# logan-pearce/olpefit

Hardware: NVIDIA B200
Metric: pixel_model_evals_per_sec (higher is better)
Workload: dtype f32

## Files before the change

### olpefit_b200/csrc/lapf.cu

```cuda
#include <algorithm>
#include <charconv>
#include <cmath>
#include <cstdarg>
#include <cstdio>
#include <cstdlib>
#include <cstring>
#include <limits>
#include <new>
#include <string>
#include <vector>

#include <cuda.h>

#include "../../include/lapf.h"
#include "lapf_device.cuh"

using namespace lapf;

static thread_local char g_err[512] = "";

static int fail(int code, const char* fmt, ...) {
    va_list ap;
    va_start(ap, fmt);
    vsnprintf(g_err, sizeof(g_err), fmt, ap);
// ... 410 lines not shown
        if (u == next_rec) {
            if (lane <= P && tw == 0) {
                const size_t mi = (size_t)wl * (P + 1) + lane;
                const double v = (lane == P) ? chi_c : p;
                const double dl = v - a.shift[mi];
                if (a.chain) {
                    const size_t ci = ((size_t)row * a.n_walkers + wl) * (P + 1) + lane;
                    if (a.chain_f32) static_cast<float*>(a.chain)[ci] = (float)dl; else static_cast<double*>(a.chain)[ci] = v;
                }
                atomicAdd(&a.moments[2 * mi], dl);
                atomicAdd(&a.moments[2 * mi + 1], dl * dl);
            }
            if (a.sk_hist) {
                double xy[2 * NB];
#pragma unroll
                for (int j = 0; j < 2 * NB; ++j) xy[j] = shfl_f64(p, j);
                if (lane == 0 && tw == 0) record_sketch<NB>(a, wl, frame, xy);
            }
            ++row;
            next_rec += a.thin;
        }
    }

    if (tw == 0) {
        if (lane < P) st[lane] = p;
        if (lane == P) st[P] = chi_c;
        if (lane == 0) a.exps[wl] += n_exps;
    }
}

template <int NB, int NX, int NY, int NW, int MINB, int TEAM>
__global__ void __launch_bounds__(NW * 32, MINB) gibbs_kernel(const __grid_constant__ RunArgs a) {
    static_assert(NW % TEAM == 0 && (TEAM == 1 || NW / TEAM <= 15), "teams must tile the CTA (named barriers 1..15)");
    extern __shared__ __align__(128) unsigned char smem_raw[];
    __shared__ WarpScratch scratch[NW];
    __shared__ double team_part[NW / TEAM][2 * TEAM];
    __shared__ uint64_t bar;
    float* sd = reinterpret_cast<float*>(smem_raw);
    float* sw = sd + NX * NY;
    float* rt = sw + NX * NY;
    const int warp = threadIdx.x >> 5, lane = threadIdx.x & 31;

    if (threadIdx.x == 0) mbar_init(&bar, 1);
    __syncthreads();

    const int i0 = (int)(((int64_t)a.n_items * blockIdx.x) / gridDim.x);
    const int i1 = (int)(((int64_t)a.n_items * (blockIdx.x + 1)) / gridDim.x);
    int cur_frame = -1;
    uint32_t phase = 0;
    for (int it = i0; it < i1; ++it) {
        const int f = a.item_frame[it];
        if (f != cur_frame) {
            __syncthreads();
            if (threadIdx.x == 0) {
                constexpr uint32_t kBytes = NX * NY * sizeof(float);
                fence_proxy_async();
                mbar_expect_tx(&bar, 2 * kBytes);
                tma_bulk_g2s(sd, a.data + (size_t)f * NX * NY, kBytes, &bar);
                tma_bulk_g2s(sw, a.weight + (size_t)f * NX * NY, kBytes, &bar);
            }
            mbar_wait(&bar, phase);
            phase ^= 1u;
            cur_frame = f;
            prep_stamp(sd, sw, NX * NY);
            __syncthreads();
        }
        const int team = warp / TEAM, tw = warp % TEAM;
        if (team < a.item_count[it]) {
            using S = Scratch<NB, NX, NY, TEAM>;
            float* base = rt + team * (TEAM > 1 ? S::TEAM_FLOATS : S::FLOATS);
            run_walker<NB, NX, NY, TEAM>(a, sd, sw, scratch[warp], base + (TEAM > 1 ? tw * S::TAB : 0), base + TEAM * S::TAB,
                                         team_part[team], team, tw, a.walker_of[a.item_first[it] + team], f, lane);
        }
    }
}

template <int NB, int NX, int NY, int LW, int TM, int WPP>
__device__ __forceinline__ void run_batch(const RunArgs& a, const float* sd, const float* sw, float* rt, float* img,
                                          int wl, int nl, int la, int frame0, int frame1, int slot, int lane,
                                          uint32_t tmem, uint32_t slot_cols) {
    using L = Layout<NB>;
    using I = CoefImg<NB, Geo<NX>::PANELS>;
    constexpr int P = L::P;
    const bool mine = wl >= 0;
    const uint64_t gid = (uint64_t)(a.id_base + (int64_t)wl * a.id_stride);
    const bool two = TM == 1 && frame1 >= 0;
    const int ox0 = a.origin[2 * frame0], oy0 = a.origin[2 * frame0 + 1];
    const int ox1 = two ? a.origin[2 * frame1] : ox0, oy1 = two ? a.origin[2 * frame1 + 1] : oy0;
    double* st = a.state + (size_t)(mine ? wl : 0) * (P + 1);
    double chi_c = mine ? st[P] : 0.0;

    const int n_upd = (int)a.n_updates;
    int next_rec = (int)min(a.next_record - a.t0 - 1, (int64_t)0x7fffffff);
    int row = 0;
    unsigned long long n_exps = 0;

#pragma unroll 1
    for (int u = 0; u < n_upd; ++u) {
        int k = 0;
        double nv = 0.0, lnu = 0.0;
        bool skip = false;
        if (mine) {
            const Draw dr = make_draw(a.seed, gid, (uint64_t)(a.t0 + u), P);
            const double oxd = (double)((two && slot) ? ox1 : ox0), oyd = (double)((two && slot) ? oy1 : oy0);
            k = dr.k;
            lnu = dr.lnu;
            const double wz = __dmul_rn(a.widths[k], dr.z);
            const bool is_log = (a.log_mask >> k) & 1u;
            double v[P];
#pragma unroll
            for (int j = 0; j < P; ++j) v[j] = st[j];
            double pk = v[0];
#pragma unroll
            for (int j = 1; j < P; ++j) pk = (j == k) ? v[j] : pk;
            nv = is_log ? (pk < 0.0 ? nan("") : __dmul_rn(pk, exp10(wz))) : __dadd_rn(pk, wz);
#pragma unroll
            for (int j = 0; j < P; ++j) v[j] = (j == k) ? nv : v[j];
            double fl = v[2 * NB];
#pragma unroll
            for (int j = 2 * NB + 1; j < P; ++j) fl = (j == a.floor_index) ? v[j] : fl;
            Coef<NB> cf;
            coef_from_vector<NB>(cf, v, fl, oxd, oyd);
            set_fast_serial<NB, NX, NY>(cf);
            if (a.plain) cf.fast = false;
            if (NX >= 64 && a.cull) set_cull_serial<NB, NX, NY>(cf); else no_cull<NB, NX, NY>(cf);
            skip = nv != nv;
            if (skip && WPP > 1) cf.fast = true;
            store_coef<NB, Geo<NX>::PANELS>(img + lane * I::STRIDE, cf, slot | (skip ? 2 : 0));
        }
        __syncwarp();

        double chi_t = 0.0;
        if constexpr (WPP == 1) {
#pragma unroll 1
            for (int i = 0; i < nl; ++i) {
                Coef<NB> cf;
                int sl = 0;
                load_coef<NB, Geo<NX>::PANELS>(cf, img + i * I::STRIDE, &sl);
                if (sl & 2) continue;
                unsigned e_upd = 0;
                const double c = warp_chi2<NB, NX, NY, false, true, 1, TM>(cf, rt, sd, sw, nullptr, lane, 0, &e_upd,
                                                                           TM == 1 ? tmem + (uint32_t)(sl & 1) * slot_cols : tmem);
                if (lane == i) { chi_t = c; n_exps += e_upd; }
            }
        } else {
#pragma unroll 1
            for (int seg = 0; seg < 2; ++seg) {
                const int i0 = seg ? la : 0, i1 = seg ? nl : la;
#pragma unroll 1
                for (int i = i0; i < i1; i += 2) {
                    const int mine_i = min(i + (lane >> 4), i1 - 1);
                    Coef<NB> cf;
                    int sl = 0;
                    load_coef<NB, 1>(cf, img + mine_i * I::STRIDE, &sl);
                    if (__all_sync(kFull, (sl & 2) != 0)) continue;
                    sl = __shfl_sync(kFull, sl, 0) & 1;
                    unsigned e_upd = 0;
                    const double c = warp_chi2_pair<NB, NX, NY, false, true, TM>(cf, rt, sd, sw, nullptr, lane, &e_upd,
                                                                                 tmem + (uint32_t)sl * slot_cols);
                    const double c0 = shfl_f64(c, 0), c1 = shfl_f64(c, 16);
                    const unsigned e0 = __shfl_sync(kFull, e_upd, 0), e1 = __shfl_sync(kFull, e_upd, 16);
                    if (lane == i) { chi_t = c0; n_exps += e0; }
                    if (lane == i + 1 && i + 1 < i1) { chi_t = c1; n_exps += e1; }
                }
            }
        }
        __syncwarp();

        if (mine) {
            if (skip) chi_t = nan("");
            if (a.outside) {
                double fl = st[a.floor_index];
                if (k == a.floor_index) fl = nv;
                chi_t += outside_chi2(a.outside, (two && slot) ? frame1 : frame0, fl);
            }
            const bool acc = lnu < -0.5 * (chi_t - chi_c);
            atomicAdd(&a.tries[(size_t)wl * P + k], 1u);
            if (acc) {
                atomicAdd(&a.accepts[(size_t)wl * P + k], 1u);
                st[k] = nv;
                chi_c = chi_t;
            }
        }
        if (u == next_rec) {
            if (mine) {
#pragma unroll 1
                for (int j = 0; j <= P; ++j) {
                    const size_t mi = (size_t)wl * (P + 1) + j;
                    const double v = (j == P) ? chi_c : st[j];
                    const double dl = v - a.shift[mi];
                    if (a.chain) {
                        const size_t ci = ((size_t)row * a.n_walkers + wl) * (P + 1) + j;
                        if (a.chain_f32) static_cast<float*>(a.chain)[ci] = (float)dl; else static_cast<double*>(a.chain)[ci] = v;
                    }
                    atomicAdd(&a.moments[2 * mi], dl);
                    atomicAdd(&a.moments[2 * mi + 1], dl * dl);
                }
                if (a.sk_hist) {
                    double xy[2 * NB];
#pragma unroll
                    for (int j = 0; j < 2 * NB; ++j) xy[j] = st[j];
                    record_sketch<NB>(a, wl, (two && slot) ? frame1 : frame0, xy);
                }
                if (a.probe) {
                    double* pb = a.probe + ((size_t)row * a.n_walkers + wl) * 3;
                    pb[0] = (double)k; pb[1] = nv; pb[2] = chi_t;
                }
            }
            ++row;
            next_rec += a.thin;
        }
    }
    if (mine) {
        st[P] = chi_c;
        a.exps[wl] += n_exps;
    }
// ... 1349 lines not shown
```

### olpefit_b200/csrc/lapf_device.cuh

```cuda
#pragma once
#ifndef LAPF_LOOP_UNROLL
#define LAPF_LOOP_UNROLL 2
#endif
#include <cstdint>
#include <cuda_runtime.h>

namespace lapf {

constexpr float kLog2e = 1.4426950408889634f;
constexpr int kLoopUnroll = LAPF_LOOP_UNROLL;
constexpr unsigned kFull = 0xffffffffu;

template <int NB>
struct Layout {
    static constexpr int NOBJ = NB;
    static constexpr int P = 3 * NB + 10;
    static constexpr int K = 2 * NB;
    static constexpr int I_DX = 2 * NB, I_DY = 2 * NB + 1;
    static constexpr int I_AMP = 2 * NB + 2;
    static constexpr int I_RATIO = 3 * NB + 2, I_BKGD = 3 * NB + 3;
    static constexpr int I_SX = 3 * NB + 4, I_SY = 3 * NB + 5, I_SX2 = 3 * NB + 6, I_SY2 = 3 * NB + 7;
    static constexpr int I_TH = 3 * NB + 8, I_TH2 = 3 * NB + 9;
};

__device__ __forceinline__ float ex2_approx(float x) {
    float y;
    asm("ex2.approx.ftz.f32 %0, %1;" : "=f"(y) : "f"(x));
    return y;
}

__device__ __forceinline__ double shfl_f64(double v, int src) {
    int lo = __double2loint(v), hi = __double2hiint(v);
    lo = __shfl_sync(kFull, lo, src);
    hi = __shfl_sync(kFull, hi, src);
    return __hiloint2double(hi, lo);
}

__device__ __forceinline__ double shfl_xor_f64(double v, int mask) {
    int lo = __double2loint(v), hi = __double2hiint(v);
    lo = __shfl_xor_sync(kFull, lo, mask);
    hi = __shfl_xor_sync(kFull, hi, mask);
    return __hiloint2double(hi, lo);
}

__device__ __forceinline__ double warp_sum_f64(double v) {
#pragma unroll
    for (int off = 16; off >= 1; off >>= 1) v += shfl_xor_f64(v, off);
    return v;
}

__device__ __forceinline__ uint32_t smem_u32(const void* p) {
    return static_cast<uint32_t>(__cvta_generic_to_shared(p));
}
__device__ __forceinline__ void mbar_init(uint64_t* bar, uint32_t count) {
    asm volatile("mbarrier.init.shared::cta.b64 [%0], %1;" ::"r"(smem_u32(bar)), "r"(count));
    asm volatile("fence.mbarrier_init.release.cluster;" ::: "memory");
}
__device__ __forceinline__ void mbar_expect_tx(uint64_t* bar, uint32_t bytes) {
    asm volatile("mbarrier.arrive.expect_tx.shared::cta.b64 _, [%0], %1;" ::"r"(smem_u32(bar)), "r"(bytes)
                 : "memory");
}
__device__ __forceinline__ void mbar_wait(uint64_t* bar, uint32_t parity) {
    asm volatile(
        "{\n\t"
        ".reg .pred p;\n\t"
        "WAIT_%=:\n\t"
        "mbarrier.try_wait.parity.shared::cta.b64 p, [%0], %1;\n\t"
        "@p bra DONE_%=;\n\t"
        "bra WAIT_%=;\n\t"
        "DONE_%=:\n\t"
        "}" ::"r"(smem_u32(bar)),
        "r"(parity)
        : "memory");
}
__device__ __forceinline__ void tma_bulk_g2s(void* dst_smem, const void* src_gmem, uint32_t bytes,
                                             uint64_t* bar) {
    asm volatile(
        "cp.async.bulk.shared::cluster.global.mbarrier::complete_tx::bytes [%0], [%1], %2, [%3];" ::"r"(
            smem_u32(dst_smem)),
        "l"(src_gmem), "r"(bytes), "r"(smem_u32(bar))
        : "memory");
}
__device__ __forceinline__ void fence_proxy_async() {
    asm volatile("fence.proxy.async.shared::cta;" ::: "memory");
}

__device__ __forceinline__ void tmem_alloc(uint32_t* slot_in_smem, uint32_t ncols) {
    asm volatile("tcgen05.alloc.cta_group::1.sync.aligned.shared::cta.b32 [%0], %1;" ::"r"(smem_u32(slot_in_smem)), "r"(ncols)
                 : "memory");
    asm volatile("tcgen05.relinquish_alloc_permit.cta_group::1.sync.aligned;" ::: "memory");
}
__device__ __forceinline__ void tmem_dealloc(uint32_t base, uint32_t ncols) {
    asm volatile("tcgen05.dealloc.cta_group::1.sync.aligned.b32 %0, %1;" ::"r"(base), "r"(ncols) : "memory");
}
__device__ __forceinline__ void tmem_fence_before_sync() { asm volatile("tcgen05.fence::before_thread_sync;" ::: "memory"); }
__device__ __forceinline__ void tmem_fence_after_sync() { asm volatile("tcgen05.fence::after_thread_sync;" ::: "memory"); }
__device__ __forceinline__ void tmem_wait_st() { asm volatile("tcgen05.wait::st.sync.aligned;" ::: "memory"); }

__device__ __forceinline__ void tmem_st16(uint32_t addr, const float (&v)[16]) {
    asm volatile("tcgen05.st.sync.aligned.32x32b.x16.b32 [%0], {%1,%2,%3,%4,%5,%6,%7,%8,%9,%10,%11,%12,%13,%14,%15,%16};"
                 ::"r"(addr), "r"(__float_as_uint(v[0])), "r"(__float_as_uint(v[1])), "r"(__float_as_uint(v[2])),
                   "r"(__float_as_uint(v[3])), "r"(__float_as_uint(v[4])), "r"(__float_as_uint(v[5])),
                   "r"(__float_as_uint(v[6])), "r"(__float_as_uint(v[7])), "r"(__float_as_uint(v[8])),
                   "r"(__float_as_uint(v[9])), "r"(__float_as_uint(v[10])), "r"(__float_as_uint(v[11])),
                   "r"(__float_as_uint(v[12])), "r"(__float_as_uint(v[13])), "r"(__float_as_uint(v[14])),
                   "r"(__float_as_uint(v[15]))
                 : "memory");
}
__device__ __forceinline__ void tmem_ld16_issue(uint32_t addr, uint32_t (&r)[16]) {
    asm volatile("tcgen05.ld.sync.aligned.32x32b.x16.b32 {%0,%1,%2,%3,%4,%5,%6,%7,%8,%9,%10,%11,%12,%13,%14,%15}, [%16];"
                 : "=r"(r[0]), "=r"(r[1]), "=r"(r[2]), "=r"(r[3]), "=r"(r[4]), "=r"(r[5]), "=r"(r[6]), "=r"(r[7]),
                   "=r"(r[8]), "=r"(r[9]), "=r"(r[10]), "=r"(r[11]), "=r"(r[12]), "=r"(r[13]), "=r"(r[14]), "=r"(r[15])
                 : "r"(addr));
}
__device__ __forceinline__ void tmem_st8(uint32_t addr, const float (&v)[8]) {
    asm volatile("tcgen05.st.sync.aligned.32x32b.x8.b32 [%0], {%1,%2,%3,%4,%5,%6,%7,%8};"
                 ::"r"(addr), "r"(__float_as_uint(v[0])), "r"(__float_as_uint(v[1])), "r"(__float_as_uint(v[2])),
                   "r"(__float_as_uint(v[3])), "r"(__float_as_uint(v[4])), "r"(__float_as_uint(v[5])),
                   "r"(__float_as_uint(v[6])), "r"(__float_as_uint(v[7]))
                 : "memory");
}
__device__ __forceinline__ void tmem_ld8_issue(uint32_t addr, uint32_t (&r)[16]) {
    asm volatile("tcgen05.ld.sync.aligned.32x32b.x8.b32 {%0,%1,%2,%3,%4,%5,%6,%7}, [%8];"
                 : "=r"(r[8]), "=r"(r[9]), "=r"(r[10]), "=r"(r[11]), "=r"(r[12]), "=r"(r[13]), "=r"(r[14]), "=r"(r[15])
                 : "r"(addr));
}
__device__ __forceinline__ void tmem_ld8_wait(uint32_t (&r)[16]) {
    asm volatile("tcgen05.wait::ld.sync.aligned;"
                 : "+r"(r[8]), "+r"(r[9]), "+r"(r[10]), "+r"(r[11]), "+r"(r[12]), "+r"(r[13]), "+r"(r[14]), "+r"(r[15]));
}
__device__ __forceinline__ void tmem_ld16_wait(uint32_t (&r)[16]) {
    asm volatile("tcgen05.wait::ld.sync.aligned;"
                 : "+r"(r[0]), "+r"(r[1]), "+r"(r[2]), "+r"(r[3]), "+r"(r[4]), "+r"(r[5]), "+r"(r[6]), "+r"(r[7]),
                   "+r"(r[8]), "+r"(r[9]), "+r"(r[10]), "+r"(r[11]), "+r"(r[12]), "+r"(r[13]), "+r"(r[14]), "+r"(r[15]));
}

template <int NB>
struct Coef {
    static constexpr int K = 2 * NB;
    float x0[K], y0[K], amp[K];
    float sa[2], sb[2], sc[2];
    float floor;
    int seg[2][4];
    unsigned nexp;
    bool fast;
};

template <int NB>
__device__ __forceinline__ void set_shape_sc(Coef<NB>& cf, int which, float sx, float sy, float s, float c) {
    const float ivx = __fdiv_rn(1.0f, __fmul_rn(sx, sx)), ivy = __fdiv_rn(1.0f, __fmul_rn(sy, sy));
    const float cc = __fmul_rn(c, c), ss = __fmul_rn(s, s);
    cf.sa[which] = __fmul_rn(-0.5f * kLog2e, __fmaf_rn(cc, ivx, __fmul_rn(ss, ivy)));
    cf.sb[which] = __fmul_rn(__fmul_rn(-kLog2e, __fmul_rn(s, c)), __fsub_rn(ivx, ivy));
    cf.sc[which] = __fmul_rn(-0.5f * kLog2e, __fmaf_rn(ss, ivx, __fmul_rn(cc, ivy)));
}

template <int NB>
__device__ __forceinline__ void set_shape(Coef<NB>& cf, int which, float sx, float sy, float th) {
    float s, c;
    sincosf(th, &s, &c);
    set_shape_sc<NB>(cf, which, sx, sy, s, c);
}

template <int NB>
__device__ __forceinline__ void stage_trial(float* tf, int lane, double mine, double oxd, double oyd) {
    using L = Layout<NB>;
    const double dxv = shfl_f64(mine, L::I_DX), dyv = shfl_f64(mine, L::I_DY);
    __syncwarp();
    if (lane < 2 * NB) {
        const double base = mine - ((lane & 1) ? oyd : oxd);
        tf[lane] = (float)base;
        tf[L::P + lane] = (float)(base + ((lane & 1) ? dyv : dxv));
    } else if (lane < L::P) {
        tf[lane] = (float)mine;
    }
    __syncwarp();
}

template <int NB>
__device__ __forceinline__ void load_centres_amps(Coef<NB>& cf, const float* tf) {
    using L = Layout<NB>;
    const float ratio = tf[L::I_RATIO], bkgd = tf[L::I_BKGD];
#pragma unroll
    for (int o = 0; o < NB; ++o) {
        cf.x0[2 * o] = tf[2 * o];
        cf.y0[2 * o] = tf[2 * o + 1];
        cf.x0[2 * o + 1] = tf[L::P + 2 * o];
        cf.y0[2 * o + 1] = tf[L::P + 2 * o + 1];
        const float a = __fsub_rn(tf[L::I_AMP + o], bkgd);
        const float aw = __fmul_rn(a, ratio);
        cf.amp[2 * o] = __fsub_rn(a, aw);
        cf.amp[2 * o + 1] = aw;
    }
}

template <int NB>
__device__ __forceinline__ void load_shape(Coef<NB>& cf, int which, const float* tf) {
    using L = Layout<NB>;
    if (which)
        set_shape<NB>(cf, 1, tf[L::I_SX2], tf[L::I_SY2], tf[L::I_TH2]);
    else
        set_shape<NB>(cf, 0, tf[L::I_SX], tf[L::I_SY], tf[L::I_TH]);
}

template <int NB, int PANELS>
struct CoefImg {
    static constexpr int K = 2 * NB;
    static constexpr int WORDS = 3 * K + 7 + 4 * PANELS + 3;
    static constexpr int V4 = ((WORDS + 3) / 4) | 1;
    static constexpr int STRIDE = 4 * V4;
};

template <int NB, int PANELS>
__device__ __forceinline__ void store_coef(float* __restrict__ dst, const Coef<NB>& cf, int slot = 0) {
    constexpr int K = 2 * NB;
    using I = CoefImg<NB, PANELS>;
    float v[I::STRIDE];
#pragma unroll
    for (int i = 0; i < I::STRIDE; ++i) v[i] = 0.f;
#pragma unroll
    for (int k = 0; k < K; ++k) { v[k] = cf.x0[k]; v[K + k] = cf.y0[k]; v[2 * K + k] = cf.amp[k]; }
#pragma unroll
    for (int c = 0; c < 2; ++c) { v[3 * K + c] = cf.sa[c]; v[3 * K + 2 + c] = cf.sb[c]; v[3 * K + 4 + c] = cf.sc[c]; }
    v[3 * K + 6] = cf.floor;
#pragma unroll
    for (int p = 0; p < PANELS; ++p)
#pragma unroll
        for (int q = 0; q < 4; ++q) v[3 * K + 7 + 4 * p + q] = __int_as_float(cf.seg[p][q]);
    v[3 * K + 7 + 4 * PANELS] = __uint_as_float(cf.nexp);
    v[3 * K + 8 + 4 * PANELS] = __int_as_float(cf.fast ? 1 : 0);
    v[3 * K + 9 + 4 * PANELS] = __int_as_float(slot);
#pragma unroll
    for (int q = 0; q < I::V4; ++q)
        reinterpret_cast<float4*>(dst)[q] = make_float4(v[4 * q], v[4 * q + 1], v[4 * q + 2], v[4 * q + 3]);
}

template <int NB, int PANELS>
__device__ __forceinline__ void load_coef(Coef<NB>& cf, const float* __restrict__ src, int* slot = nullptr) {
    constexpr int K = 2 * NB;
    using I = CoefImg<NB, PANELS>;
    float v[I::STRIDE];
#pragma unroll
    for (int q = 0; q < I::V4; ++q) {
        const float4 t = reinterpret_cast<const float4*>(src)[q];
        v[4 * q] = t.x; v[4 * q + 1] = t.y; v[4 * q + 2] = t.z; v[4 * q + 3] = t.w;
    }
#pragma unroll
    for (int k = 0; k < K; ++k) { cf.x0[k] = v[k]; cf.y0[k] = v[K + k]; cf.amp[k] = v[2 * K + k]; }
#pragma unroll
    for (int c = 0; c < 2; ++c) { cf.sa[c] = v[3 * K + c]; cf.sb[c] = v[3 * K + 2 + c]; cf.sc[c] = v[3 * K + 4 + c]; }
    cf.floor = v[3 * K + 6];
#pragma unroll
    for (int p = 0; p < PANELS; ++p)
#pragma unroll
        for (int q = 0; q < 4; ++q) cf.seg[p][q] = __float_as_int(v[3 * K + 7 + 4 * p + q]);
    cf.nexp = __float_as_uint(v[3 * K + 7 + 4 * PANELS]);
    cf.fast = __float_as_int(v[3 * K + 8 + 4 * PANELS]) != 0;
    if (slot) *slot = __float_as_int(v[3 * K + 9 + 4 * PANELS]);
}

template <int NB>
__device__ __forceinline__ void coef_from_vector(Coef<NB>& cf, const double (&v)[Layout<NB>::P], double floor_v,
                                                 double oxd, double oyd) {
    using L = Layout<NB>;
    float tf[L::P + 2 * NB];
#pragma unroll
    for (int j = 0; j < L::P; ++j) {
        if (j < 2 * NB) {
            const double base = v[j] - ((j & 1) ? oyd : oxd);
            tf[j] = (float)base;
            tf[L::P + j] = (float)(base + ((j & 1) ? v[L::I_DY] : v[L::I_DX]));
        } else {
            tf[j] = (float)v[j];
        }
    }
    load_centres_amps<NB>(cf, tf);
    cf.floor = (float)floor_v;
    set_shape<NB>(cf, 0, tf[L::I_SX], tf[L::I_SY], tf[L::I_TH]);
    set_shape<NB>(cf, 1, tf[L::I_SX2], tf[L::I_SY2], tf[L::I_TH2]);
}

template <int NX, int WPP = 1>
struct Geo {
    static constexpr int PW = NX >= 64 ? 64 : 32;
    static constexpr int PANELS = NX / PW;
    static constexpr int GPR = PW / 4;
    static constexpr int LPW = 32 / WPP;
    static constexpr int BPS = LPW / GPR;
    static constexpr int RG = 2 * BPS;
    static_assert(NX % PW == 0 && (NX == 32 || NX % 64 == 0), "unsupported stamp width");
    static_assert(WPP == 1 || (WPP == 2 && NX == 32), "two vectors per pass: 32-pixel stamps only");
};

template <int NB>
struct Tab {
    static constexpr int K = 2 * NB;
    static constexpr int RS = 28;
    static constexpr int OFF_T = 2 * K;
    static_assert(OFF_T + 16 <= RS && OFF_T % 4 == 0, "block table entry layout");
};

template <int NY, int TEAM = 1>
struct Rows {
    static constexpr int TR = NY < 64 ? NY : 64;
    static constexpr int HALVES = NY / TR;
    static constexpr int NBLK = TR / 2 / TEAM;
    static_assert(NY % TR == 0 && (TR / 2) % TEAM == 0, "unsupported stamp height");
};

template <int NB, int NX, int NY, int TEAM = 1, int WPP = 1>
struct Scratch {
    static constexpr int TEAM_NBLK = NY * Geo<NX>::PANELS / (2 * TEAM);
    static constexpr int TAB1 = (TEAM > 1 ? TEAM_NBLK : Rows<NY, TEAM>::NBLK) * Tab<NB>::RS + (WPP > 1 ? 8 : 0);
    static constexpr int TAB = WPP * TAB1;
    static constexpr int CT = 2 * NB * 2 * Geo<NX>::GPR * 4;
    static constexpr int FLOATS = TAB + WPP * CT;
    static constexpr int TEAM_FLOATS = TEAM * TAB + Geo<NX>::PANELS * CT;
};

template <int NB, int NX, int TR, int TEAM, int WPP = 1>
__device__ __forceinline__ void build_row_table(float* __restrict__ rt, const Coef<NB>& cf, int lane, int row0, int tw) {
    using G = Geo<NX, WPP>;
    using T = Tab<NB>;
    constexpr int K = 2 * NB;
    constexpr int NQ = K / 2;
    constexpr int NBLK = TR / 2 / TEAM;
#ifdef LAPF_EXP_SPLIT
    constexpr int SPLIT = NBLK >= 32 ? 1 : (NBLK >= 16 ? 2 : (TEAM == 1 ? 2 : 4));
#else
    constexpr int SPLIT = (TEAM == 1 || NBLK >= 32) ? 1 : (NBLK >= 16 ? 2 : 4);
#endif
    __syncwarp();
    if (WPP > 1) rt += (lane / G::LPW) * (NBLK * T::RS + 8);
#pragma unroll
    for (int j0 = 0; j0 < NBLK * SPLIT; j0 += G::LPW) {
        const int idx = j0 + lane % G::LPW;
        if ((NBLK * SPLIT) % G::LPW == 0 || idx < NBLK * SPLIT) {
            const int jb = idx / SPLIT, part = idx % SPLIT;
            const int step = (jb / G::BPS) * TEAM + tw;
            const float yb = (float)(row0 + step * G::RG + 2 * (jb % G::BPS)) + 0.5f;
            float4* o = reinterpret_cast<float4*>(rt + jb * T::RS);
#pragma unroll
            for (int q0 = 0; q0 < NQ; q0 += SPLIT) {
                const int q = q0 + part;
                if (NQ % SPLIT == 0 || q < NQ) {
                    float y0a = cf.y0[2 * q0], y0b = cf.y0[2 * q0 + 1];
#pragma unroll
                    for (int t = 1; t < SPLIT; ++t)
                        if (q0 + t < NQ && part == t) { y0a = cf.y0[2 * (q0 + t)]; y0b = cf.y0[2 * (q0 + t) + 1]; }
                    const float yda = __fsub_rn(yb, y0a), ydb = __fsub_rn(yb, y0b);
                    o[q] = make_float4(__fmul_rn(cf.sb[0], yda), __fmul_rn(__fmul_rn(cf.sc[0], yda), yda),
                                       __fmul_rn(cf.sb[1], ydb), __fmul_rn(__fmul_rn(cf.sc[1], ydb), ydb));
                }
            }
            const float2 jlo = make_float2(-1.5f, -0.5f), jhi = make_float2(0.5f, 1.5f);
#pragma unroll
            for (int p0 = 0; p0 < 4; p0 += SPLIT) {
                const int pr = p0 + part;
                const bool c = (pr >> 1) != 0, hi = (pr & 1) != 0;
                const float sbc = c ? cf.sb[1] : cf.sb[0], scc = c ? cf.sc[1] : cf.sc[0];
                const float yd = __fsub_rn(yb, c ? cf.y0[1] : cf.y0[0]);
                const float p = __fmul_rn(sbc, yd);
                const float sy = __fmul_rn(__fmul_rn(scc, yd), 2.f);
                const float g = __fmul_rn(0.25f, scc);
                const float i = hi ? 0.5f : -0.5f;
                const float pj = __fmaf_rn(i, sbc, p), base = __fmaf_rn(i, sy, g);
                const float2 pj2 = make_float2(pj, pj), b2 = make_float2(base, base);
                const float2 alo = __ffma2_rn(jlo, pj2, b2), ahi = __ffma2_rn(jhi, pj2, b2);
                o[T::OFF_T / 4 + pr] = make_float4(ex2_approx(alo.x), ex2_approx(alo.y), ex2_approx(ahi.x), ex2_approx(ahi.y));
            }
        }
    }
    __syncwarp();
}

template <int NX, int NY>
__device__ __forceinline__ void cull_one(float a, float x0, float y0, float sa, float sb, float sc, float floor_v,
                                         int& lo, int& hi, uint32_t& pm) {
    using G = Geo<NX>;
    constexpr int STEPS = NY / G::RG;
    constexpr uint32_t kAllPans = (1u << G::PANELS) - 1u;
    const float tau = __fmul_rn(0x1p-27f, fabsf(floor_v));
    const float L = __log2f(__fdividef(fabsf(a), tau));
    lo = 0; hi = STEPS - 1;
    pm = kAllPans;
    if (L <= 0.f) {
        lo = STEPS; hi = -1; pm = 0u;
    } else {
        const float sb2 = __fmul_rn(sb, sb);
        const float ky = __fsub_rn(sc, __fdividef(sb2, __fmul_rn(4.f, sa))), kx = __fsub_rn(sa, __fdividef(sb2, __fmul_rn(4.f, sc)));
        const float Y = __fadd_rn(__fsqrt_rn(__fdividef(L, -ky)), 1.f), X = __fadd_rn(__fsqrt_rn(__fdividef(L, -kx)), 1.f);
        if (Y < 1e6f && fabsf(y0) < 1e6f) {
            constexpr float kInvRG = 1.f / (float)G::RG;
            lo = max(0, (int)ceilf(__fmul_rn(__fsub_rn(__fsub_rn(y0, Y), (float)(G::RG - 1)), kInvRG)));
            hi = min(STEPS - 1, (int)floorf(__fmul_rn(__fadd_rn(y0, Y), kInvRG)));
            if (lo > hi) { lo = STEPS; hi = -1; }
        }
        if (G::PANELS > 1 && X < 1e6f && fabsf(x0) < 1e6f) {
            pm = 0u;
#pragma unroll
            for (int p = 0; p < G::PANELS; ++p)
                if (__fadd_rn(x0, X) >= (float)(p * G::PW) && __fsub_rn(x0, X) <= (float)(p * G::PW + G::PW - 1)) pm |= 1u << p;
        }
    }
}

template <int NB, int NX, int NY, int TEAM>
__device__ __forceinline__ void set_segments(Coef<NB>& cf, const int (&lo)[2], const int (&hi)[2], const uint32_t (&pm)[2]) {
    using G = Geo<NX>;
    constexpr int STEPS = NY / G::RG;
    unsigned n = 0;
#pragma unroll
    for (int pan = 0; pan < G::PANELS; ++pan) {
        const bool n_on = ((pm[0] >> pan) & 1u) && lo[0] <= hi[0];
        const bool w_on = ((pm[1] >> pan) & 1u) && lo[1] <= hi[1];
        int nlo = n_on ? lo[0] : STEPS, nhi1 = n_on ? hi[0] + 1 : STEPS;
        int wlo = w_on ? lo[1] : nlo, whi1 = w_on ? hi[1] + 1 : nhi1;
        wlo = min(wlo, nlo);
        whi1 = max(whi1, nhi1);
        if (!n_on) { nlo = whi1; nhi1 = whi1; }
        if (!cf.fast || TEAM > 1) { wlo = 0; nlo = 0; nhi1 = STEPS; whi1 = STEPS; }
        cf.seg[pan][0] = wlo; cf.seg[pan][1] = nlo; cf.seg[pan][2] = nhi1; cf.seg[pan][3] = whi1;
        n += (unsigned)((nhi1 - nlo) + (whi1 - wlo));
    }
    cf.nexp = (unsigned)(G::PW * G::RG * NB) * n;
}

template <int NB, int NX, int NY, int TEAM = 1>
__device__ __forceinline__ void set_cull(Coef<NB>& cf, int lane) {
    using G = Geo<NX>;
    constexpr int K = 2 * NB;
    constexpr int STEPS = NY / G::RG;
    float a = cf.amp[0], x0 = cf.x0[0], y0 = cf.y0[0];
#pragma unroll
    for (int k = 1; k < K; ++k)
// ... 247 lines not shown
        if (TASKS % (TEAM * 32) == 0 || t < TASKS) {
            const int a = t % G::GPR, kk = (t / G::GPR) % K, pan = t / (G::GPR * K);
            float amp = cf.amp[0], x0 = cf.x0[0], y0 = cf.y0[0];
#pragma unroll
            for (int k = 1; k < K; ++k)
                if (kk == k) { amp = cf.amp[k]; x0 = cf.x0[k]; y0 = cf.y0[k]; }
            const int c = kk & 1;
            const float sa = c ? cf.sa[1] : cf.sa[0], sb = c ? cf.sb[1] : cf.sb[0], sc = c ? cf.sc[1] : cf.sc[0];
            const float dy0 = (c ? cf.y0[1] : cf.y0[0]) - y0;
            float4 lo, hi;
            block_consts(amp, ((float)(pan * G::PW + 4 * a) + 1.5f) - x0, dy0, sa, sb, sc, lo, hi);
            float4* base = reinterpret_cast<float4*>(ct) + pan * (K * 2 * G::GPR);
            base[(kk * 2) * G::GPR + a] = lo;
            base[(kk * 2 + 1) * G::GPR + a] = hi;
        }
    }
}

template <int NB, int NX>
__device__ __forceinline__ void own_consts(LaneK<NB>& lk, const Coef<NB>& cf, int lane, int pan) {
    using G = Geo<NX>;
    constexpr int K = 2 * NB;
    const float xa = (float)(pan * G::PW + 4 * (lane % G::GPR)) + 1.5f;
#pragma unroll
    for (int k = 0; k < K; ++k) {
        const int c = k & 1;
        lk.dxa[k] = xa - cf.x0[k];
        float4 lo, hi;
        block_consts(cf.amp[k], lk.dxa[k], cf.y0[c] - cf.y0[k], cf.sa[c], cf.sb[c], cf.sc[c], lo, hi);
        lk.C[k][0] = make_float2(lo.x, lo.y); lk.C[k][1] = make_float2(lo.z, lo.w);
        lk.C[k][2] = make_float2(hi.x, hi.y); lk.C[k][3] = make_float2(hi.z, hi.w);
    }
}

template <int NB, int NX>
__device__ __forceinline__ void read_consts(LaneK<NB>& lk, const float* __restrict__ ct, const Coef<NB>& cf, int lane, int pan) {
    using G = Geo<NX>;
    constexpr int K = 2 * NB;
    const int mine = lane % G::GPR;
    const float xa = (float)(pan * G::PW + 4 * mine) + 1.5f;
#pragma unroll
    for (int k = 0; k < K; ++k) {
#pragma unroll
        for (int ii = 0; ii < 2; ++ii) {
            const float4 v = reinterpret_cast<const float4*>(ct)[(k * 2 + ii) * G::GPR + mine];
            lk.C[k][2 * ii] = make_float2(v.x, v.y);
            lk.C[k][2 * ii + 1] = make_float2(v.z, v.w);
        }
        lk.dxa[k] = xa - cf.x0[k];
    }
}

template <int NB, int NX, int NY, bool STORE, bool PREP, int KIND, int TM = 0, int WPP = 1>
__device__ __forceinline__ void row_steps_fast(const Coef<NB>& cf, const LaneK<NB>& lk, float2& s0, float2& s1,
                                               int& i, int i1, StepPtrs& sp, bool keep = true) {
    using G = Geo<NX, WPP>;
    using T = Tab<NB>;
    constexpr int K = 2 * NB;
    const float* rp = sp.rp;
    const float* dp = sp.dp;
    const float* wp = sp.wp;
    float* mp = sp.mp;
    uint32_t tm = sp.tm;
#pragma unroll kLoopUnroll
    for (; i < i1; ++i) {
        float4 d0, d1, w0, w1;
        uint32_t tv[16];
        if (TM == 1) {
            tmem_ld16_issue(tm, tv);
        } else if (TM == 2) {
            tmem_ld8_issue(tm, tv);
            d0 = *reinterpret_cast<const float4*>(dp);
            d1 = *reinterpret_cast<const float4*>(dp + NX);
        } else {
            d0 = *reinterpret_cast<const float4*>(dp);
            d1 = *reinterpret_cast<const float4*>(dp + NX);
            w0 = *reinterpret_cast<const float4*>(wp);
            w1 = *reinterpret_cast<const float4*>(wp + NX);
        }
        float2 m[4];
#pragma unroll
        for (int j = 0; j < 4; ++j) m[j] = make_float2(cf.floor, cf.floor);
        if (KIND > 0) {
            float rc[2 * K];
#pragma unroll
            for (int q = 0; q < 2 * K / 4; ++q) {
                const float4 t4 = reinterpret_cast<const float4*>(rp)[q];
                rc[4 * q] = t4.x; rc[4 * q + 1] = t4.y; rc[4 * q + 2] = t4.z; rc[4 * q + 3] = t4.w;
            }
#pragma unroll
            for (int c = (KIND == 2 ? 0 : 1); c < 2; ++c) {
                const float4 T0 = reinterpret_cast<const float4*>(rp + T::OFF_T)[2 * c];
                const float4 T1 = reinterpret_cast<const float4*>(rp + T::OFF_T)[2 * c + 1];
                float2 u[4];
#pragma unroll
                for (int o = 0; o < NB; ++o) {
                    const int k = 2 * o + c;
                    const float q = __fmaf_rn(lk.dxa[k], __fmaf_rn(cf.sa[c], lk.dxa[k], rc[2 * k]), rc[2 * k + 1]);
                    const float e = ex2_approx(q);
                    const float2 e2 = make_float2(e, e);
#pragma unroll
                    for (int p = 0; p < 4; ++p)
                        u[p] = (o == 0) ? __fmul2_rn(lk.C[k][p], e2) : __ffma2_rn(lk.C[k][p], e2, u[p]);
                }
                m[0] = __ffma2_rn(make_float2(T0.x, T0.y), u[0], m[0]); m[1] = __ffma2_rn(make_float2(T0.z, T0.w), u[1], m[1]);
                m[2] = __ffma2_rn(make_float2(T1.x, T1.y), u[2], m[2]); m[3] = __ffma2_rn(make_float2(T1.z, T1.w), u[3], m[3]);
            }
        }
        if (TM == 1) {
            tmem_ld16_wait(tv);
            d0 = make_float4(__uint_as_float(tv[0]), __uint_as_float(tv[1]), __uint_as_float(tv[2]), __uint_as_float(tv[3]));
            d1 = make_float4(__uint_as_float(tv[4]), __uint_as_float(tv[5]), __uint_as_float(tv[6]), __uint_as_float(tv[7]));
            tm += 16;
        } else if (TM == 2) {
            tmem_ld8_wait(tv);
            tm += 8;
        }
        if (TM) {
            w0 = make_float4(__uint_as_float(tv[8]), __uint_as_float(tv[9]), __uint_as_float(tv[10]), __uint_as_float(tv[11]));
            w1 = make_float4(__uint_as_float(tv[12]), __uint_as_float(tv[13]), __uint_as_float(tv[14]), __uint_as_float(tv[15]));
        }
        finish_step<NX, STORE, PREP>(m, d0, d1, w0, w1, mp, s0, s1, keep);
        if (STORE) mp += G::RG * NX;
        rp += G::BPS * T::RS;
        dp += G::RG * NX;
        wp += G::RG * NX;
    }
    sp.rp = rp; sp.dp = dp; sp.wp = wp; sp.mp = mp; sp.tm = tm;
}

template <int NB, int NX, int NY, bool STORE, bool PREP, int TEAM = 1, int TM = 0>
__device__ __forceinline__ double warp_chi2(const Coef<NB>& cf, float* __restrict__ scratch,
                                            const float* __restrict__ d, const float* __restrict__ w,
                                            float* __restrict__ model_out, int lane, int tw = 0,
                                            unsigned* exps = nullptr, uint32_t tmem = 0) {
    static_assert(TEAM == 1, "whole-warp passes only");
    using G = Geo<NX>;
    using T = Tab<NB>;
    using R = Rows<NY, TEAM>;
    constexpr int K = 2 * NB;
    constexpr int TR = R::TR;
    constexpr int STEPS = TR / G::RG;
    static_assert(TM == 0 || (TEAM == 1 && PREP), "the TMEM pixel store holds prepared stamps for whole-warp passes");
    static_assert(TM != 1 || (R::HALVES == 1 && G::PANELS == 1), "both planes fit the 512 TMEM columns up to 64 x 64 pixels");
    constexpr int TM_STEP = TM == 1 ? 16 : 8;
    static_assert(TR % G::RG == 0, "unsupported stamp height");
    static_assert(STEPS % TEAM == 0, "team size must divide the warp steps");
    float* rt = scratch;
    float* ct = scratch + Scratch<NB, NX, NY, TEAM>::TAB;
    const int a = lane % G::GPR, b = lane / G::GPR;
    double acc = 0.0;
    if (exps) *exps += cf.nexp;
#pragma unroll 1
    for (int half = 0; half < R::HALVES; ++half) {
        if (cf.fast) build_row_table<NB, NX, TR, TEAM>(rt, cf, lane, half * TR, tw);
#pragma unroll 1
        for (int pan = 0; pan < G::PANELS; ++pan) {
            const int off0 = (half * TR + 2 * b) * NX + pan * G::PW + 4 * a;
            const bool p1 = G::PANELS > 1 && pan > 0;
            int wlo = p1 ? cf.seg[1][0] : cf.seg[0][0], nlo = p1 ? cf.seg[1][1] : cf.seg[0][1];
            int nhi1 = p1 ? cf.seg[1][2] : cf.seg[0][2], whi1 = p1 ? cf.seg[1][3] : cf.seg[0][3];
            if (R::HALVES > 1) {
                const int base = half * STEPS;
                wlo = min(max(wlo - base, 0), STEPS); nlo = min(max(nlo - base, 0), STEPS);
                nhi1 = min(max(nhi1 - base, 0), STEPS); whi1 = min(max(whi1 - base, 0), STEPS);
            }
            float2 s0 = make_float2(0.f, 0.f), s1 = make_float2(0.f, 0.f);
            if (cf.fast) {
                LaneK<NB> lk;
                coop_consts<NB, NX>(lk, ct, cf, lane, pan);
                {
                    StepPtrs sp{rt + b * T::RS, d + off0, w + off0, STORE ? model_out + off0 : nullptr,
                                tmem + (uint32_t)((half * G::PANELS + pan) * STEPS * TM_STEP), 0.f};
                    int i = 0;
                    if (NX < 64) {
                        row_steps_fast<NB, NX, NY, STORE, PREP, 2, TM>(cf, lk, s0, s1, i, STEPS, sp);
                    } else {
                        row_steps_fast<NB, NX, NY, STORE, PREP, 0, TM>(cf, lk, s0, s1, i, wlo, sp);
                        row_steps_fast<NB, NX, NY, STORE, PREP, 1, TM>(cf, lk, s0, s1, i, nlo, sp);
                        row_steps_fast<NB, NX, NY, STORE, PREP, 2, TM>(cf, lk, s0, s1, i, nhi1, sp);
                        row_steps_fast<NB, NX, NY, STORE, PREP, 1, TM>(cf, lk, s0, s1, i, whi1, sp);
                        row_steps_fast<NB, NX, NY, STORE, PREP, 0, TM>(cf, lk, s0, s1, i, STEPS, sp);
                    }
                }
            } else {
                float2 xd[K][2];
                const float fa = (float)(pan * G::PW + 4 * a);
#pragma unroll
                for (int k = 0; k < K; ++k) {
                    const float2 nx0 = make_float2(-cf.x0[k], -cf.x0[k]);
                    xd[k][0] = __fadd2_rn(make_float2(fa, fa + 1.f), nx0);
                    xd[k][1] = __fadd2_rn(make_float2(fa + 2.f, fa + 3.f), nx0);
                }
#pragma unroll 1
                for (int mth = 0; mth < STEPS / TEAM; ++mth) {
                    const int st = mth * TEAM + tw;
                    const int so = st * G::RG * NX;
                    StepPtrs sp{nullptr, d + off0 + so, w + off0 + so, STORE ? model_out + off0 + so : nullptr,
                                TM == 1 ? tmem + (uint32_t)(st * 16) : 0u, (float)(half * TR + st * G::RG + 2 * b)};
                    int i = 0;
                    row_steps<NB, NX, NY, STORE, PREP, 1, (TM == 1 ? 1 : 0)>(cf, xd, s0, s1, i, 1, sp);
                }
            }
            acc += (double)((s0.x + s0.y) + (s1.x + s1.y));
        }
    }
    return warp_sum_f64(acc);
}

template <int NB, int NX, int NY, int TEAM>
__device__ __forceinline__ double team_chi2(const Coef<NB>& cf, float* __restrict__ rt, const float* __restrict__ d,
                                            const float* __restrict__ w, int lane, int tw, unsigned* exps,
                                            const float* __restrict__ team_ct) {
    using G = Geo<NX>;
    using T = Tab<NB>;
    constexpr int K = 2 * NB;
    constexpr int RGROUPS = TEAM / G::PANELS;
    constexpr int TSTEPS = NY / G::RG;
    constexpr int MY = TSTEPS / RGROUPS;
    static_assert(TEAM > 1 && TEAM % G::PANELS == 0 && RGROUPS > 1 && TSTEPS % RGROUPS == 0, "unsupported team size");
    static_assert(MY * G::BPS == Scratch<NB, NX, NY, TEAM>::TEAM_NBLK, "table size");
    const int pan = tw % G::PANELS, rgp = tw / G::PANELS;
    const int a = lane % G::GPR, b = lane / G::GPR;
    const int off0 = (2 * b) * NX + pan * G::PW + 4 * a;
    if (exps) *exps += cf.nexp;
    float2 s0 = make_float2(0.f, 0.f), s1 = make_float2(0.f, 0.f);
    if (cf.fast) {
        build_row_table<NB, NX, NY, RGROUPS>(rt, cf, lane, 0, rgp);
        LaneK<NB> lk;
        read_consts<NB, NX>(lk, team_ct + pan * Scratch<NB, NX, NY, TEAM>::CT, cf, lane, pan);
#pragma unroll(MY < 4 ? MY : 2)
        for (int m = 0; m < MY; ++m) {
            const int so = (m * RGROUPS + rgp) * G::RG * NX;
            StepPtrs sp{rt + (m * G::BPS + b) * T::RS, d + off0 + so, w + off0 + so, nullptr, 0u, 0.f};
            int i = 0;
            row_steps_fast<NB, NX, NY, false, true, 2>(cf, lk, s0, s1, i, 1, sp);
        }
    } else {
        float2 xd[K][2];
        const float fa = (float)(pan * G::PW + 4 * a);
#pragma unroll
        for (int k = 0; k < K; ++k) {
            const float2 nx0 = make_float2(-cf.x0[k], -cf.x0[k]);
            xd[k][0] = __fadd2_rn(make_float2(fa, fa + 1.f), nx0);
            xd[k][1] = __fadd2_rn(make_float2(fa + 2.f, fa + 3.f), nx0);
        }
#pragma unroll 1
        for (int m = 0; m < MY; ++m) {
            const int st = m * RGROUPS + rgp;
            const int so = st * G::RG * NX;
            StepPtrs sp{nullptr, d + off0 + so, w + off0 + so, nullptr, 0u, (float)(st * G::RG + 2 * b)};
            int i = 0;
            row_steps<NB, NX, NY, false, true>(cf, xd, s0, s1, i, 1, sp);
        }
    }
    return warp_sum_f64((double)((s0.x + s0.y) + (s1.x + s1.y)));
}

template <int NB, int NX, int NY, bool STORE, bool PREP, int TM = 0>
__device__ __forceinline__ double warp_chi2_pair(const Coef<NB>& cf, float* __restrict__ scratch,
                                                 const float* __restrict__ d, const float* __restrict__ w,
                                                 float* __restrict__ model_out, int lane, unsigned* exps = nullptr,
                                                 uint32_t tmem = 0) {
    using G = Geo<NX, 2>;
    using T = Tab<NB>;
    using S = Scratch<NB, NX, NY, 1, 2>;
    constexpr int K = 2 * NB;
    constexpr int STEPS = NY / G::RG;
    static_assert(NX == 32 && NY == 32 && G::PANELS == 1, "two vectors per pass: 32 x 32 stamps");
    static_assert(TM == 0 || PREP, "the TMEM pixel store holds prepared stamps");
    const int wl = lane % G::LPW, h = lane / G::LPW, a = wl % G::GPR, b = wl / G::GPR;
    float* rt = scratch;
    float* ct = scratch + S::TAB;
    if (exps) *exps += cf.nexp;
    const bool run_fast = __any_sync(kFull, cf.fast), run_plain = __any_sync(kFull, !cf.fast);
    const int off0 = (2 * b) * NX + 4 * a;
    float2 s0 = make_float2(0.f, 0.f), s1 = make_float2(0.f, 0.f);
    if (run_fast) {
        build_row_table<NB, NX, NY, 1, 2>(rt, cf, lane, 0, 0);
        LaneK<NB> lk;
        coop_consts<NB, NX, 2>(lk, ct, cf, lane, 0);
        float2 f0 = make_float2(0.f, 0.f), f1 = make_float2(0.f, 0.f);
        StepPtrs sp{rt + h * S::TAB1 + b * T::RS, d + off0, w + off0, STORE ? model_out + off0 : nullptr, tmem, 0.f};
        int i = 0;
        row_steps_fast<NB, NX, NY, STORE, PREP, 2, TM, 2>(cf, lk, f0, f1, i, STEPS, sp, cf.fast);
        if (cf.fast) { s0 = f0; s1 = f1; }
    }
    if (run_plain) {
        float2 xd[K][2];
        const float fa = (float)(4 * a);
// ... 122 lines not shown
```

Measured before the change: 2394 billion.

## Defer per-walker warp reductions to lane partials and reorder row-table exponent layout

```diff
diff --git a/olpefit_b200/csrc/lapf.cu b/olpefit_b200/csrc/lapf.cu
--- a/olpefit_b200/csrc/lapf.cu
+++ b/olpefit_b200/csrc/lapf.cu
@@ -516,6 +516,8 @@
     using L = Layout<NB>;
     using I = CoefImg<NB, Geo<NX>::PANELS>;
     constexpr int P = L::P;
+    constexpr bool LANE_SUMS = WPP == 1 && Geo<NX>::PANELS == 1 && Rows<NY, 1>::HALVES == 1;
+    static_assert(!LANE_SUMS || I::STRIDE >= 32, "a walker's image holds the 32 lane partials of its pass");
     const bool mine = wl >= 0;
     const uint64_t gid = (uint64_t)(a.id_base + (int64_t)wl * a.id_stride);
     const bool two = TM == 1 && frame1 >= 0;
@@ -560,12 +562,28 @@
             if (NX >= 64 && a.cull) set_cull_serial<NB, NX, NY>(cf); else no_cull<NB, NX, NY>(cf);
             skip = nv != nv;
             if (skip && WPP > 1) cf.fast = true;
+            if (LANE_SUMS && !skip) n_exps += cf.nexp;
             store_coef<NB, Geo<NX>::PANELS>(img + lane * I::STRIDE, cf, slot | (skip ? 2 : 0));
         }
         __syncwarp();
 
         double chi_t = 0.0;
-        if constexpr (WPP == 1) {
+        if constexpr (LANE_SUMS) {
+#pragma unroll 1
+            for (int i = 0; i < nl; ++i) {
+                Coef<NB> cf;
+                int sl = 0;
+                float* slot_img = img + i * I::STRIDE;
+                load_coef<NB, 1>(cf, slot_img, &sl);
+                if (sl & 2) continue;
+                __syncwarp();
+                const float part = lane_chi2<NB, NX, NY, TM>(cf, rt, sd, sw, lane,
+                                                             TM == 1 ? tmem + (uint32_t)(sl & 1) * slot_cols : tmem);
+                slot_img[lane] = part;
+            }
+            __syncwarp();
+            if (mine) chi_t = warp_sum_f64_of(img + lane * I::STRIDE);
+        } else if constexpr (WPP == 1) {
 #pragma unroll 1
             for (int i = 0; i < nl; ++i) {
                 Coef<NB> cf;
diff --git a/olpefit_b200/csrc/lapf_device.cuh b/olpefit_b200/csrc/lapf_device.cuh
--- a/olpefit_b200/csrc/lapf_device.cuh
+++ b/olpefit_b200/csrc/lapf_device.cuh
@@ -47,6 +47,21 @@
 #pragma unroll
     for (int off = 16; off >= 1; off >>= 1) v += shfl_xor_f64(v, off);
     return v;
+}
+
+__device__ __forceinline__ double warp_sum_f64_of(const float* __restrict__ p) {
+    double v[16];
+#pragma unroll
+    for (int q = 0; q < 4; ++q) {
+        const float4 a = reinterpret_cast<const float4*>(p)[q], b = reinterpret_cast<const float4*>(p)[q + 4];
+        v[4 * q] = (double)a.x + (double)b.x; v[4 * q + 1] = (double)a.y + (double)b.y;
+        v[4 * q + 2] = (double)a.z + (double)b.z; v[4 * q + 3] = (double)a.w + (double)b.w;
+    }
+#pragma unroll
+    for (int off = 8; off >= 1; off >>= 1)
+#pragma unroll
+        for (int l = 0; l < off; ++l) v[l] += v[l + off];
+    return v[0];
 }
 
 __device__ __forceinline__ uint32_t smem_u32(const void* p) {
@@ -207,7 +222,7 @@
 struct CoefImg {
     static constexpr int K = 2 * NB;
     static constexpr int WORDS = 3 * K + 7 + 4 * PANELS + 3;
-    static constexpr int V4 = ((WORDS + 3) / 4) | 1;
+    static constexpr int V4 = ((WORDS + 3) / 4 > 8 ? (WORDS + 3) / 4 : 8) | 1;
     static constexpr int STRIDE = 4 * V4;
 };
 
@@ -297,7 +312,10 @@
     static constexpr int K = 2 * NB;
     static constexpr int RS = 28;
     static constexpr int OFF_T = 2 * K;
+    static_assert(NB == 2 || NB == 3, "pieces 0, 1: class 0, 1 of objects 0 and 1; piece 2: object 2");
     static_assert(OFF_T + 16 <= RS && OFF_T % 4 == 0, "block table entry layout");
+    __host__ __device__ static constexpr int ka(int q) { return q < 2 ? q : 4; }
+    __host__ __device__ static constexpr int kb(int q) { return q < 2 ? q + 2 : 5; }
 };
 
 template <int NY, int TEAM = 1>
@@ -344,13 +362,19 @@
             for (int q0 = 0; q0 < NQ; q0 += SPLIT) {
                 const int q = q0 + part;
                 if (NQ % SPLIT == 0 || q < NQ) {
-                    float y0a = cf.y0[2 * q0], y0b = cf.y0[2 * q0 + 1];
+                    float y0a = cf.y0[T::ka(q0)], y0b = cf.y0[T::kb(q0)];
+                    float sba = cf.sb[T::ka(q0) & 1], sbb = cf.sb[T::kb(q0) & 1];
+                    float sca = cf.sc[T::ka(q0) & 1], scb = cf.sc[T::kb(q0) & 1];
 #pragma unroll
                     for (int t = 1; t < SPLIT; ++t)
-                        if (q0 + t < NQ && part == t) { y0a = cf.y0[2 * (q0 + t)]; y0b = cf.y0[2 * (q0 + t) + 1]; }
+                        if (q0 + t < NQ && part == t) {
+                            const int ka = T::ka(q0 + t), kb = T::kb(q0 + t);
+                            y0a = cf.y0[ka]; y0b = cf.y0[kb];
+                            sba = cf.sb[ka & 1]; sbb = cf.sb[kb & 1]; sca = cf.sc[ka & 1]; scb = cf.sc[kb & 1];
+                        }
                     const float yda = __fsub_rn(yb, y0a), ydb = __fsub_rn(yb, y0b);
-                    o[q] = make_float4(__fmul_rn(cf.sb[0], yda), __fmul_rn(__fmul_rn(cf.sc[0], yda), yda),
-                                       __fmul_rn(cf.sb[1], ydb), __fmul_rn(__fmul_rn(cf.sc[1], ydb), ydb));
+                    o[q] = make_float4(__fmul_rn(sba, yda), __fmul_rn(sbb, ydb),
+                                       __fmul_rn(__fmul_rn(sca, yda), yda), __fmul_rn(__fmul_rn(scb, ydb), ydb));
                 }
             }
             const float2 jlo = make_float2(-1.5f, -0.5f), jhi = make_float2(0.5f, 1.5f);
@@ -764,23 +788,29 @@
 #pragma unroll
         for (int j = 0; j < 4; ++j) m[j] = make_float2(cf.floor, cf.floor);
         if (KIND > 0) {
-            float rc[2 * K];
-#pragma unroll
-            for (int q = 0; q < 2 * K / 4; ++q) {
-                const float4 t4 = reinterpret_cast<const float4*>(rp)[q];
-                rc[4 * q] = t4.x; rc[4 * q + 1] = t4.y; rc[4 * q + 2] = t4.z; rc[4 * q + 3] = t4.w;
-            }
 #pragma unroll
             for (int c = (KIND == 2 ? 0 : 1); c < 2; ++c) {
                 const float4 T0 = reinterpret_cast<const float4*>(rp + T::OFF_T)[2 * c];
                 const float4 T1 = reinterpret_cast<const float4*>(rp + T::OFF_T)[2 * c + 1];
+                float ea[NB];
+                {
+                    const float4 r = reinterpret_cast<const float4*>(rp)[c];
+                    const float2 dx = make_float2(lk.dxa[c], lk.dxa[2 + c]);
+                    const float2 q = __ffma2_rn(dx, __ffma2_rn(make_float2(cf.sa[c], cf.sa[c]), dx, make_float2(r.x, r.y)),
+                                                make_float2(r.z, r.w));
+                    ea[0] = ex2_approx(q.x);
+                    ea[1] = ex2_approx(q.y);
+                }
+                if (NB > 2) {
+                    const float4 r = reinterpret_cast<const float4*>(rp)[2];
+                    const float dx = lk.dxa[4 + c];
+                    ea[NB - 1] = ex2_approx(__fmaf_rn(dx, __fmaf_rn(cf.sa[c], dx, c ? r.y : r.x), c ? r.w : r.z));
+                }
                 float2 u[4];
 #pragma unroll
                 for (int o = 0; o < NB; ++o) {
                     const int k = 2 * o + c;
-                    const float q = __fmaf_rn(lk.dxa[k], __fmaf_rn(cf.sa[c], lk.dxa[k], rc[2 * k]), rc[2 * k + 1]);
-                    const float e = ex2_approx(q);
-                    const float2 e2 = make_float2(e, e);
+                    const float2 e2 = make_float2(ea[o], ea[o]);
 #pragma unroll
                     for (int p = 0; p < 4; ++p)
                         u[p] = (o == 0) ? __fmul2_rn(lk.C[k][p], e2) : __ffma2_rn(lk.C[k][p], e2, u[p]);
@@ -811,6 +841,69 @@
     sp.rp = rp; sp.dp = dp; sp.wp = wp; sp.mp = mp; sp.tm = tm;
 }
 
+template <int NB, int NX, int NY, bool STORE, bool PREP, int TM = 0>
+__device__ __forceinline__ float panel_chi2(const Coef<NB>& cf, float* __restrict__ scratch,
+                                            const float* __restrict__ d, const float* __restrict__ w,
+                                            float* __restrict__ model_out, int lane, int half, int pan, uint32_t tmem) {
+    using G = Geo<NX>;
+    using T = Tab<NB>;
+    using R = Rows<NY, 1>;
+    constexpr int K = 2 * NB;
+    constexpr int TR = R::TR;
+    constexpr int STEPS = TR / G::RG;
+    static_assert(TM == 0 || PREP, "the TMEM pixel store holds prepared stamps");
+    static_assert(TM != 1 || (R::HALVES == 1 && G::PANELS == 1), "both planes fit the 512 TMEM columns up to 64 x 64 pixels");
+    constexpr int TM_STEP = TM == 1 ? 16 : 8;
+    static_assert(TR % G::RG == 0, "unsupported stamp height");
+    const float* rt = scratch;
+    float* ct = scratch + Scratch<NB, NX, NY>::TAB;
+    const int a = lane % G::GPR, b = lane / G::GPR;
+    const int off0 = (half * TR + 2 * b) * NX + pan * G::PW + 4 * a;
+    const bool p1 = G::PANELS > 1 && pan > 0;
+    int wlo = p1 ? cf.seg[1][0] : cf.seg[0][0], nlo = p1 ? cf.seg[1][1] : cf.seg[0][1];
+    int nhi1 = p1 ? cf.seg[1][2] : cf.seg[0][2], whi1 = p1 ? cf.seg[1][3] : cf.seg[0][3];
+    if (R::HALVES > 1) {
+        const int base = half * STEPS;
+        wlo = min(max(wlo - base, 0), STEPS); nlo = min(max(nlo - base, 0), STEPS);
+        nhi1 = min(max(nhi1 - base, 0), STEPS); whi1 = min(max(whi1 - base, 0), STEPS);
+    }
+    float2 s0 = make_float2(0.f, 0.f), s1 = make_float2(0.f, 0.f);
+    if (cf.fast) {
+        LaneK<NB> lk;
+        coop_consts<NB, NX>(lk, ct, cf, lane, pan);
+        StepPtrs sp{rt + b * T::RS, d + off0, w + off0, STORE ? model_out + off0 : nullptr,
+                    tmem + (uint32_t)((half * G::PANELS + pan) * STEPS * TM_STEP), 0.f};
+        int i = 0;
+        if (NX < 64) {
+            row_steps_fast<NB, NX, NY, STORE, PREP, 2, TM>(cf, lk, s0, s1, i, STEPS, sp);
+        } else {
+            row_steps_fast<NB, NX, NY, STORE, PREP, 0, TM>(cf, lk, s0, s1, i, wlo, sp);
+            row_steps_fast<NB, NX, NY, STORE, PREP, 1, TM>(cf, lk, s0, s1, i, nlo, sp);
+            row_steps_fast<NB, NX, NY, STORE, PREP, 2, TM>(cf, lk, s0, s1, i, nhi1, sp);
+            row_steps_fast<NB, NX, NY, STORE, PREP, 1, TM>(cf, lk, s0, s1, i, whi1, sp);
+            row_steps_fast<NB, NX, NY, STORE, PREP, 0, TM>(cf, lk, s0, s1, i, STEPS, sp);
+        }
+    } else {
+        float2 xd[K][2];
+        const float fa = (float)(pan * G::PW + 4 * a);
+#pragma unroll
+        for (int k = 0; k < K; ++k) {
+            const float2 nx0 = make_float2(-cf.x0[k], -cf.x0[k]);
+            xd[k][0] = __fadd2_rn(make_float2(fa, fa + 1.f), nx0);
+            xd[k][1] = __fadd2_rn(make_float2(fa + 2.f, fa + 3.f), nx0);
+        }
+#pragma unroll 1
+        for (int st = 0; st < STEPS; ++st) {
+            const int so = st * G::RG * NX;
+            StepPtrs sp{nullptr, d + off0 + so, w + off0 + so, STORE ? model_out + off0 + so : nullptr,
+                        TM == 1 ? tmem + (uint32_t)(st * 16) : 0u, (float)(half * TR + st * G::RG + 2 * b)};
+            int i = 0;
+            row_steps<NB, NX, NY, STORE, PREP, 1, (TM == 1 ? 1 : 0)>(cf, xd, s0, s1, i, 1, sp);
+        }
+    }
+    return (s0.x + s0.y) + (s1.x + s1.y);
+}
+
 template <int NB, int NX, int NY, bool STORE, bool PREP, int TEAM = 1, int TM = 0>
 __device__ __forceinline__ double warp_chi2(const Coef<NB>& cf, float* __restrict__ scratch,
                                             const float* __restrict__ d, const float* __restrict__ w,
@@ -818,76 +911,25 @@
                                             unsigned* exps = nullptr, uint32_t tmem = 0) {
     static_assert(TEAM == 1, "whole-warp passes only");
     using G = Geo<NX>;
-    using T = Tab<NB>;
     using R = Rows<NY, TEAM>;
-    constexpr int K = 2 * NB;
-    constexpr int TR = R::TR;
-    constexpr int STEPS = TR / G::RG;
-    static_assert(TM == 0 || (TEAM == 1 && PREP), "the TMEM pixel store holds prepared stamps for whole-warp passes");
-    static_assert(TM != 1 || (R::HALVES == 1 && G::PANELS == 1), "both planes fit the 512 TMEM columns up to 64 x 64 pixels");
-    constexpr int TM_STEP = TM == 1 ? 16 : 8;
-    static_assert(TR % G::RG == 0, "unsupported stamp height");
-    static_assert(STEPS % TEAM == 0, "team size must divide the warp steps");
-    float* rt = scratch;
-    float* ct = scratch + Scratch<NB, NX, NY, TEAM>::TAB;
-    const int a = lane % G::GPR, b = lane / G::GPR;
     double acc = 0.0;
     if (exps) *exps += cf.nexp;
 #pragma unroll 1
     for (int half = 0; half < R::HALVES; ++half) {
-        if (cf.fast) build_row_table<NB, NX, TR, TEAM>(rt, cf, lane, half * TR, tw);
+        if (cf.fast) build_row_table<NB, NX, R::TR, TEAM>(scratch, cf, lane, half * R::TR, tw);
 #pragma unroll 1
-        for (int pan = 0; pan < G::PANELS; ++pan) {
-            const int off0 = (half * TR + 2 * b) * NX + pan * G::PW + 4 * a;
-            const bool p1 = G::PANELS > 1 && pan > 0;
-            int wlo = p1 ? cf.seg[1][0] : cf.seg[0][0], nlo = p1 ? cf.seg[1][1] : cf.seg[0][1];
-            int nhi1 = p1 ? cf.seg[1][2] : cf.seg[0][2], whi1 = p1 ? cf.seg[1][3] : cf.seg[0][3];
-            if (R::HALVES > 1) {
-                const int base = half * STEPS;
-                wlo = min(max(wlo - base, 0), STEPS); nlo = min(max(nlo - base, 0), STEPS);
-                nhi1 = min(max(nhi1 - base, 0), STEPS); whi1 = min(max(whi1 - base, 0), STEPS);
-            }
-            float2 s0 = make_float2(0.f, 0.f), s1 = make_float2(0.f, 0.f);
-            if (cf.fast) {
-                LaneK<NB> lk;
-                coop_consts<NB, NX>(lk, ct, cf, lane, pan);
-                {
-                    StepPtrs sp{rt + b * T::RS, d + off0, w + off0, STORE ? model_out + off0 : nullptr,
-                                tmem + (uint32_t)((half * G::PANELS + pan) * STEPS * TM_STEP), 0.f};
-                    int i = 0;
-                    if (NX < 64) {
-                        row_steps_fast<NB, NX, NY, STORE, PREP, 2, TM>(cf, lk, s0, s1, i, STEPS, sp);
-                    } else {
-                        row_steps_fast<NB, NX, NY, STORE, PREP, 0, TM>(cf, lk, s0, s1, i, wlo, sp);
-                        row_steps_fast<NB, NX, NY, STORE, PREP, 1, TM>(cf, lk, s0, s1, i, nlo, sp);
-                        row_steps_fast<NB, NX, NY, STORE, PREP, 2, TM>(cf, lk, s0, s1, i, nhi1, sp);
-                        row_steps_fast<NB, NX, NY, STORE, PREP, 1, TM>(cf, lk, s0, s1, i, whi1, sp);
-                        row_steps_fast<NB, NX, NY, STORE, PREP, 0, TM>(cf, lk, s0, s1, i, STEPS, sp);
-                    }
-                }
-            } else {
-                float2 xd[K][2];
-                const float fa = (float)(pan * G::PW + 4 * a);
-#pragma unroll
-                for (int k = 0; k < K; ++k) {
-                    const float2 nx0 = make_float2(-cf.x0[k], -cf.x0[k]);
-                    xd[k][0] = __fadd2_rn(make_float2(fa, fa + 1.f), nx0);
-                    xd[k][1] = __fadd2_rn(make_float2(fa + 2.f, fa + 3.f), nx0);
-                }
-#pragma unroll 1
-                for (int mth = 0; mth < STEPS / TEAM; ++mth) {
-                    const int st = mth * TEAM + tw;
-                    const int so = st * G::RG * NX;
-                    StepPtrs sp{nullptr, d + off0 + so, w + off0 + so, STORE ? model_out + off0 + so : nullptr,
-                                TM == 1 ? tmem + (uint32_t)(st * 16) : 0u, (float)(half * TR + st * G::RG + 2 * b)};
-                    int i = 0;
-                    row_steps<NB, NX, NY, STORE, PREP, 1, (TM == 1 ? 1 : 0)>(cf, xd, s0, s1, i, 1, sp);
-                }
-            }
-            acc += (double)((s0.x + s0.y) + (s1.x + s1.y));
-        }
+        for (int pan = 0; pan < G::PANELS; ++pan)
+            acc += (double)panel_chi2<NB, NX, NY, STORE, PREP, TM>(cf, scratch, d, w, model_out, lane, half, pan, tmem);
     }
     return warp_sum_f64(acc);
+}
+
+template <int NB, int NX, int NY, int TM>
+__device__ __forceinline__ float lane_chi2(const Coef<NB>& cf, float* __restrict__ scratch, const float* __restrict__ d,
+                                           const float* __restrict__ w, int lane, uint32_t tmem) {
+    static_assert(Geo<NX>::PANELS == 1 && Rows<NY, 1>::HALVES == 1, "one table, one panel");
+    if (cf.fast) build_row_table<NB, NX, NY, 1>(scratch, cf, lane, 0, 0);
+    return panel_chi2<NB, NX, NY, false, true, TM>(cf, scratch, d, w, nullptr, lane, 0, 0, tmem);
 }
 
 template <int NB, int NX, int NY, int TEAM>
```

After: 2476 billion, median of 6. 3.4% higher.
